# sailist/emotion-recognition-in-conversation

Measured on AMD Instinct MI355X. Metric: utterances/sec training step, COGMEN IEMOCAP-6 atv, higher is better.
Workload: dtype bf16

## Files before the change

emotion-recognition-in-conversation_amd/csrc/cogmen_fused.hip:

```cpp
#include "erc_common.h"
#include "split_dev.h"
#include "store_dev.h"

namespace {

typedef float f32x4 __attribute__((ext_vector_type(4)));
typedef short bf16x8 __attribute__((ext_vector_type(8)));

constexpr int CG_F = 100;
constexpr int CG_R = 8;
constexpr int CG_HL = 5;
constexpr int CG_TR = 16;
constexpr int CG_MID = CG_TR + 2 * CG_HL;
constexpr int CG_OUT = CG_TR + 4 * CG_HL;
constexpr int CG_FAR = CG_TR + 6 * CG_HL;
constexpr int CG_KM = (CG_R + 1) * CG_F;
constexpr int CG_KMP = 928;
constexpr int CG_SM = 936;
constexpr int CG_SH1 = 136;
constexpr int CG_SQ = 404;
constexpr int CG_CH = 12;
constexpr int CG_NT = 7;

constexpr int CG_NW = 16;
// ... 533 lines not shown
#pragma unroll
                for (int kb = 0; kb < 4; ++kb) {
                    sp_u32x4 fa0[NT], fa1[NT], fb[NT];
#pragma unroll
                    for (int t = 0; t < NT; ++t) {
                        const unsigned short* const pl = sH1 + t * (FW_SH1_BYTES / 2) + 32 * kb + 8 * g;
                        fa0[t] = *reinterpret_cast<const sp_u32x4*>(pl + r * CG_SH1), fa1[t] = *reinterpret_cast<const sp_u32x4*>(pl + (16 + r) * CG_SH1);
                        fb[t] = fqx[kb][t];
                        if (j == 0 && NT == 2) fqx[kb][t] = *reinterpret_cast<const sp_u32x4*>(bq1 + t * p.q_plane + 512 * kb);
                    }
                    acc[0] = sp_mfma<NT>(fa0, fb, acc[0]);
                    acc[1] = sp_mfma<NT>(fa1, fb, acc[1]);
                }
                if (j == 0 && NT > 2) {
                    __builtin_amdgcn_sched_barrier(0);
#pragma unroll
                    for (int kb = 0; kb < 4; ++kb)
#pragma unroll
                        for (int t = 0; t < NT; ++t) fqx[kb][t] = *reinterpret_cast<const sp_u32x4*>(bq1 + t * p.q_plane + 512 * kb);
                }
            } else {
#pragma unroll
            for (int kb = 0; kb < 4; ++kb)
#pragma unroll
                for (int h = 0; h < 2; ++h) acc[h] = __builtin_amdgcn_mfma_f32_16x16x32_bf16(fa[h][kb], fq[j][kb], acc[h], 0, 0, 0);
            }
            if (qt < 25) {
#pragma unroll
                for (int h = 0; h < 2; ++h)
#pragma unroll
                    for (int i = 0; i < 4; ++i) {
                        const int e = 16 * h + 4 * g + i;
                        if (e < CG_MID) sQ[e * CG_SQ + 16 * qt + r] = acc[h][i] + qbias[j];
                    }
            }
        }
    }
    __syncthreads();
    CG_STAMP(4);

#pragma unroll
    for (int j = 0; j < 2; ++j) {
        const int i = tid + CG_NTH * j;
        const int li = i / 100, q = i % 100;
        const int node = r0 + li;
        if (i < CG_TR * 100 && node < N)
            st_out16(p.QKVS + (int64_t)node * 400 + 4 * q, *reinterpret_cast<const f32x4*>(sQ + (CG_HL + li) * CG_SQ + 4 * q), p.wt);
    }

    {
        const bool act = lane < CG_F / 2;
        const int c2 = 2 * min(lane, CG_F / 2 - 1);
        const float am = act ? 1.f : 0.f;
        const int li = w, node = r0 + li, e = CG_HL + li;
        const bool valid = node < N;
        const int e0 = __builtin_amdgcn_readfirstlane(max(sIp[e] - E_lo, 0));
        const int nwin = __builtin_amdgcn_readfirstlane(valid ? min(max(sIp[e + 1] - sIp[e], 0), CG_CH) : 0);
        float2 qv = *reinterpret_cast<const float2*>(sQ + e * CG_SQ + c2);
        qv.x *= am, qv.y *= am;
        const float2 sk = *reinterpret_cast<const float2*>(sQ + e * CG_SQ + 3 * CG_F + c2);
        int ljs[CG_CH];
#pragma unroll
        for (int u = 0; u < CG_CH; ++u) ljs[u] = closed ? sSrc[e] + min(u, max(nwin - 1, 0)) : sSrc[min(e0 + min(u, max(nwin - 1, 0)), FW_ECAP - 1)];
        float2 kv[CG_CH], vv[CG_CH];
#pragma unroll
        for (int u = 0; u < CG_CH; ++u) {
            const float* row = sQ + min(max(ljs[u] - mb, 0), CG_MID - 1) * CG_SQ;
            kv[u] = *reinterpret_cast<const float2*>(row + CG_F + c2), vv[u] = *reinterpret_cast<const float2*>(row + 2 * CG_F + c2);
        }
        float sc[CG_CH], part[16];
#pragma unroll
        for (int u = 0; u < 16; ++u) part[u] = u < CG_CH ? qv.x * kv[u < CG_CH ? u : 0].x + qv.y * kv[u < CG_CH ? u : 0].y : 0.f;
        wave_sums_ch(part, sc, lane);
        float mx = -INFINITY, den = 0.f, o0 = 0.f, o1 = 0.f;
#pragma unroll
        for (int u = 0; u < CG_CH; ++u) {
            sc[u] *= p.scale;
            if (u < nwin) mx = fmaxf(mx, sc[u]);
        }
#pragma unroll
        for (int u = 0; u < CG_CH; ++u) {
            const float pw = u < nwin ? expf(sc[u] - mx) : 0.f;
            sc[u] = pw;
            den += pw;
            o0 += pw * vv[u].x, o1 += pw * vv[u].y;
        }
        const float inv = 1.0f / (den + 1e-16f);
        const float2 y = make_float2(valid ? o0 * inv + sk.x : 0.f, valid ? o1 * inv + sk.y : 0.f);
        if (act) *reinterpret_cast<float2*>(sH2 + li * CG_F + c2) = y;
        if (valid) {
            if (act && !p.h2_rows) *reinterpret_cast<float2*>(p.H2 + (int64_t)node * p.ldh2 + c2) = y;
            float mine = 0.f;
#pragma unroll
            for (int u = 0; u < CG_CH; ++u)
                if (lane == u) mine = sc[u];
            if (lane < nwin) p.alpha[sIp[e] + lane] = mine * inv;
        }
    }
    CG_STAMP(5);
    if (!p.bn_fused) return;

    __syncthreads();
    if (p.h2_rows && tid >= 512 && tid < 512 + CG_TR * (CG_F / 4)) {
        const int li = (tid - 512) / (CG_F / 4), q = (tid - 512) % (CG_F / 4);
        const int node = r0 + li;
        if (node < N) st_out16(p.H2 + (int64_t)node * p.ldh2 + 4 * q, *reinterpret_cast<const f32x4*>(sH2 + li * CG_F + 4 * q), p.wt);
    }
    if (tid < 2 * CG_F) {
        const int c = tid % CG_F, sq = tid / CG_F;
        double s = 0.0;
#pragma unroll
        for (int li = 0; li < CG_TR; ++li) {
            const double x = (double)sH2[li * CG_F + c];
            s += sq ? x * x : x;
        }
        if (p.bn_fused == 2) {
            reinterpret_cast<float*>(p.bn_part)[(int64_t)blockIdx.x * 2 * CG_F + tid] = (float)s;
        } else {
            st_sc1d(p.bn_part + (int64_t)blockIdx.x * 2 * CG_F + tid, s);
        }
    }
    if (p.bn_fused == 2) {
        CG_STAMP(6);
        return;
    }
    asm volatile("s_waitcnt vmcnt(0)" ::: "memory");
    __syncthreads();
    CG_STAMP(6);
    if (tid == 0) {
        const int prev = __hip_atomic_fetch_add(p.bn_counter, 1, __ATOMIC_RELAXED, __HIP_MEMORY_SCOPE_AGENT);
        const int last = prev == (int)gridDim.x - 1;
        if (last) __hip_atomic_store(p.bn_counter, 0, __ATOMIC_RELAXED, __HIP_MEMORY_SCOPE_AGENT);
        *s_last = last;
    }
    __syncthreads();
    if (!*s_last) return;
    {
        const int slot = tid & 255, part = tid >> 8;
        const int G = (int)gridDim.x, Gq = (G + 3) >> 2;
        const int g_begin = min(part * Gq, G), g_end = min(G, g_begin + Gq);
        double s = 0.0;
        if (slot < 2 * CG_F) {
            for (int g0 = g_begin; g0 < g_end; g0 += 32) {
                double t[32];
#pragma unroll
                for (int j = 0; j < 32; ++j) t[j] = ld_sc1d(p.bn_part + (int64_t)min(g0 + j, G - 1) * 2 * CG_F + slot);
#pragma unroll
                for (int j = 0; j < 32; ++j) s += t[j] * (g0 + j < g_end ? 1.0 : 0.0);
            }
        }
        sRed[part * 256 + slot] = s;
        __syncthreads();
        if (tid < CG_F) {
            const int c = tid;
            const double sx = ((sRed[c] + sRed[256 + c]) + sRed[512 + c]) + sRed[768 + c];
            const double sxx = ((sRed[CG_F + c] + sRed[256 + CG_F + c]) + sRed[512 + CG_F + c]) + sRed[768 + CG_F + c];
            const double m = sx / (double)N;
            double var = sxx / (double)N - m * m;
            if (var < 0.0) var = 0.0;
            p.saved[c] = (float)m;
            p.saved[CG_F + c] = (float)(1.0 / sqrt(var + (double)p.eps));
            const double unbiased = N > 1 ? var * (double)N / (double)(N - 1) : var;
            p.running_mean[c] = (1.f - p.momentum) * p.running_mean[c] + p.momentum * (float)m;
            p.running_var[c] = (1.f - p.momentum) * p.running_var[c] + p.momentum * (float)unbiased;
        }
        if (p.stamps && tid == 0) p.stamps[7] = __builtin_amdgcn_s_memrealtime();
    }
}

template <int CTRL>
__device__ __forceinline__ float cg_dpp(float v) {
    return __builtin_bit_cast(float, __builtin_amdgcn_update_dpp(0, __builtin_bit_cast(int, v), CTRL, 0xF, 0xF, true));
}
__device__ __forceinline__ float cg_row16_sum(float v) {
    v += cg_dpp<0xB1>(v), v += cg_dpp<0x4E>(v), v += cg_dpp<0x141>(v), v += cg_dpp<0x140>(v);
    return v;
}

constexpr int BW_ROWS = 48;
constexpr int BW_SK_OFF = 0;
constexpr int BW_SK_BYTES = BW_ROWS * CG_F * 4;
constexpr int BW_SV_OFF = BW_SK_OFF + BW_SK_BYTES;
constexpr int BW_SQ_OFF = BW_SV_OFF + BW_SK_BYTES;
constexpr int BW_SQ_BYTES = BW_ROWS * CG_F * 4;
constexpr int BW_BAND = 68;
constexpr int BW_SG_OFF = BW_SQ_OFF + BW_SQ_BYTES;
constexpr int BW_SE_OFF = BW_SG_OFF + BW_SQ_BYTES;
constexpr int BW_ECAP = 400;
constexpr int BW_OCAP = 288;
constexpr int BW_SE_BYTES = (3 * BW_ECAP + 4 * BW_OCAP + 40 + 28) * 4;
constexpr int BW_SDQ_OFF = BW_SE_OFF + ((BW_SE_BYTES + 15) / 16) * 16;
constexpr int CG_SDQ = 424;
constexpr int BW_SDQ_BYTES = 32 * CG_SDQ * 2;
constexpr int BW_SDH1_OFF = BW_SDQ_OFF + BW_SDQ_BYTES;
constexpr int BW_SDH1_BYTES = 32 * CG_F * 4;
constexpr int BW_SDP_OFF = BW_SDH1_OFF + BW_SDH1_BYTES;
constexpr int BW_SDP_BYTES = CG_TR * 968 * 2;
constexpr int BW_LDS = BW_SDP_OFF + BW_SDP_BYTES;
constexpr int CG_KB = 936;
constexpr int CG_KBP = 960;
constexpr int CG_SDP = 968;
static_assert(CG_TR * CG_SDP * 2 <= BW_SDP_BYTES && BW_SDP_OFF % 16 == 0 && BW_LDS <= 160 * 1024, "backward LDS map");
static_assert(2 * BW_ROWS * BW_BAND * 4 <= BW_SDP_BYTES, "the two band matrices live in the dP tile's area until the dP stage");
static_assert(3 * 4 * 2 * 64 * 4 * 4 <= BW_SDQ_BYTES, "K-split partials of the band product live in the dQKVS tile's area");

constexpr int BX_DQ_ROWS = CG_MID + 1;
constexpr int BX_DQPLANE = BX_DQ_ROWS * CG_SDQ * 2;
constexpr int BX_CP = 528;
constexpr int BX_DPPLANE = CG_TR * BX_CP * 2;
constexpr int BX_ZERO = 2 * 520;
template <int NT> constexpr int BX_PF = 3;
constexpr int BX_SE_BYTES16 = ((BW_SE_BYTES + 15) / 16) * 16;
template <int NT>
struct BxMap {
    static constexpr int SK_OFF = 0, SQ_OFF = BW_SK_BYTES, SG_OFF = 2 * BW_SK_BYTES;
    static constexpr int SE_OFF = 3 * BW_SK_BYTES;
    static constexpr int BAND_OFF = SE_OFF + BX_SE_BYTES16;
    static constexpr int BAND_BYTES = 2 * BW_ROWS * BW_BAND * 4;
    static constexpr int SV_OFF = BAND_OFF + BAND_BYTES;
    static constexpr int E_OFF = SV_OFF + BW_SK_BYTES;
    static constexpr int E_BYTES = NT * BX_DQPLANE - BW_SK_BYTES > 24576 ? NT * BX_DQPLANE - BW_SK_BYTES : 24576;
    static constexpr int LUT_OFF = E_OFF + E_BYTES;
    static constexpr int LDS = LUT_OFF + 1024;
    static_assert(NT * BX_DPPLANE <= 3 * BW_SK_BYTES && BW_SDH1_BYTES + 7 * 64 * 4 * 4 <= BAND_BYTES && LDS <= 160 * 1024 && SV_OFF % 16 == 0 &&
                      E_OFF % 16 == 0, "split backward LDS map");
};

struct CgBwdP {
    const float* dY;
    const float* H2;
    const float* gamma;
    const float* saved;
    const float* bn_bwd;
    const float* QKVS;
    const float* alpha;
    const int32_t* in_ptr;
    const int32_t* in_src;
    const int32_t* out_ptr;
    const int32_t* out_dst;
    const int32_t* out_typ;
    const int32_t* out_eid;
    const float* inv_cnt;
    const int32_t* node_spk;
    const float* head_part;
    float* bn_bwd_out;
    float* dgamma;
    float* dbeta;
    float* stats;
    int head_parts, hp_floats;
    const unsigned short* WqT;
    const unsigned short* Wb;
    float* dQKVS;
    float* dH1;
    float* dH0;
    float scale;
    int N, ldh2, lddh0, lddh1, grads_bf16, two_spk;
    const int32_t* n_dev;
    uint64_t* stamps;
    int stamp_block;
    int64_t qT_plane, wb_plane;
    int wt, dq_rows, dh1_rows;
    const int32_t* node_rec;
    int wp, wf;
};

template <int NT, bool CL>
__global__ __launch_bounds__(CG_NTH) void cogmen_bwd_tile_kernel(const CgBwdP p) {
    constexpr bool X = NT > 1;
    using XM = BxMap<X ? NT : 2>;
    extern __shared__ __attribute__((aligned(16))) unsigned char lds[];
    float* const sK = reinterpret_cast<float*>(lds + (X ? XM::SK_OFF : BW_SK_OFF));
    float* const sV = reinterpret_cast<float*>(lds + (X ? XM::SV_OFF : BW_SV_OFF));
    float* const sQq = reinterpret_cast<float*>(lds + (X ? XM::SQ_OFF : BW_SQ_OFF));
    float* const sG = reinterpret_cast<float*>(lds + (X ? XM::SG_OFF : BW_SG_OFF));
    float* const sAl = reinterpret_cast<float*>(lds + (X ? XM::SE_OFF : BW_SE_OFF));
    int* const sSrc = reinterpret_cast<int*>(sAl + 2 * BW_ECAP);
    int* const sOd = sSrc + BW_ECAP;
    int* const sOt = sOd + 2 * BW_OCAP;
    float* const sOw = reinterpret_cast<float*>(sOt + BW_OCAP);
    int* const sIp = reinterpret_cast<int*>(sOw + BW_OCAP);
    int* const sOp = sIp + 40;
    int* const sSpkOwn = reinterpret_cast<int*>(sAl + BW_ECAP);
    unsigned short* const sDQ = reinterpret_cast<unsigned short*>(lds + (X ? XM::SV_OFF : BW_SDQ_OFF));
    float* const sDH1 = reinterpret_cast<float*>(lds + (X ? XM::BAND_OFF : BW_SDH1_OFF));
    unsigned short* const sDP = reinterpret_cast<unsigned short*>(lds + (X ? XM::SK_OFF : BW_SDP_OFF));
    float* const sPart3 = sK;
    float* const sPart5 = X ? reinterpret_cast<float*>(lds + XM::BAND_OFF + BW_SDH1_BYTES) : sG;
    uint32_t* const sLut = reinterpret_cast<uint32_t*>(lds + XM::LUT_OFF);
    const int tid = threadIdx.x, lane = tid & 63, r = lane & 15, g = lane >> 4;
    const int w = __builtin_amdgcn_readfirstlane(tid >> 6);
    const int N = p.n_dev ? min(max(*p.n_dev, 1), p.N) : p.N;
    const int r0 = (int)blockIdx.x * CG_TR;
    const int mb = r0 - CG_HL, ob = r0 - 2 * CG_HL, fb = r0 - 3 * CG_HL;
    const int c1 = min(lane + 64, CG_F - 1);
    const bool h1 = lane + 64 < CG_F;
    const int ct = w & 7, kh = w >> 3;
    const bool mma_wave = ct < CG_NT;
    CG_STAMP(0);

    const int o_lo_node = min(max(ob, 0), N), o_hi_node = min(max(ob + CG_OUT, 0), N);
    const int m_lo_node = min(max(mb, 0), N), m_hi_node = min(max(mb + CG_MID, 0), N);
    constexpr bool closed = CL;
    int E_lo, E_hi, O_lo = 0, O_hi = 0;
    if constexpr (closed) {
        E_lo = p.node_rec[4 * (int64_t)o_lo_node + 2], E_hi = min(p.node_rec[4 * (int64_t)o_hi_node + 2], E_lo + BW_ECAP);
        if (tid < CG_OUT + 1) {
            const int nc = min(max(ob + tid, 0), N);
            const int4 rec = *reinterpret_cast<const int4*>(p.node_rec + 4 * (int64_t)nc);
            sIp[tid] = rec.z, sSrc[tid] = nc - min(rec.x, p.wf), sOd[tid] = rec.x, sOd[64 + tid] = rec.y;
        }
        if (tid >= 64 && tid < 64 + CG_OUT) {
            const int node = ob + tid - 64;
            const int sp = p.node_spk[min(max(node, 0), N - 1)];
            sOt[tid - 64] = (node >= 0 && node < N) ? sp : -1;
        }
    } else {
        E_lo = p.in_ptr[o_lo_node], E_hi = min(p.in_ptr[o_hi_node], E_lo + BW_ECAP);
        O_lo = p.out_ptr[m_lo_node], O_hi = min(p.out_ptr[m_hi_node], O_lo + BW_OCAP);
        if (tid < CG_OUT + 1) sIp[tid] = p.in_ptr[min(max(ob + tid, 0), N)];
        if (tid >= 64 && tid < 64 + CG_MID + 1) sOp[tid - 64] = p.out_ptr[min(max(mb + tid - 64, 0), N)];
    }
    if (tid >= 128 && tid < 128 + CG_TR) sSpkOwn[tid - 128] = p.node_spk[min(r0 + tid - 128, N - 1)];
    double* const sHp = reinterpret_cast<double*>(lds + (X ? XM::E_OFF : BW_SDQ_OFF));
    float* const sBnB = reinterpret_cast<float*>(lds + (X ? XM::E_OFF : BW_SDQ_OFF) + 4 * 256 * 8);
    if constexpr (X) {
        if (tid >= 768 && tid < 1024) {
            const int k4 = 4 * (tid - 768), q = k4 / 104, within = k4 - q * 104;
            uint32_t e = 3u << 16;
            if (q < CG_R) e = (uint32_t)(2 * ((q & 3) * 104 + within)) | ((1u + (uint32_t)(q >> 2)) << 16);
            else if (q == CG_R) e = (uint32_t)(2 * (4 * 104 + within));
            sLut[tid - 768] = e;
        }
    }
    if (p.head_part) {
        const int slot = tid & 255, part = tid >> 8;
        const int G = p.head_parts, Gq = (G + 3) >> 2;
        const int g_begin = min(part * Gq, G), g_end = min(G, g_begin + Gq);
        double acc = 0.0;
        if (slot < p.hp_floats) {
            for (int g0 = g_begin; g0 < g_end; g0 += 16) {
                float t[16];
#pragma unroll
                for (int j = 0; j < 16; ++j) t[j] = p.head_part[(int64_t)min(g0 + j, G - 1) * p.hp_floats + slot];
#pragma unroll
                for (int j = 0; j < 16; ++j) acc += (double)t[j] * (g0 + j < g_end ? 1.0 : 0.0);
            }
        }
        sHp[part * 256 + slot] = acc;
    }
    {
#pragma unroll
        for (int j = 0; j < 3; ++j) {
            const int i = tid + CG_NTH * j;
            const int f = min(i / 50, BW_ROWS - 1), q = i % 50;
            const int node = fb + f;
            const bool ok = f < CG_FAR && node >= 0 && node < N;
            const f32x4 v = *reinterpret_cast<const f32x4*>(p.QKVS + (int64_t)min(max(node, 0), N - 1) * 400 + CG_F + 4 * q);
            const float m = ok ? 1.f : 0.f;
            float* dst = (q < 25 ? sK + f * CG_F + 4 * q : sV + f * CG_F + 4 * (q - 25));
            if (i < BW_ROWS * 50) *reinterpret_cast<f32x4*>(dst) = (f32x4){v.x * m, v.y * m, v.z * m, v.w * m};
        }
        if (tid < BW_ECAP) {
            const int ei = min(E_lo + tid, max(E_hi - 1, E_lo));
            const bool ok = E_lo + tid < E_hi;
            const float a = p.alpha[ei];
            sAl[tid] = ok ? a : 0.f;
            if (!closed) {
                const int sj = p.in_src[ei];
                sSrc[tid] = ok ? sj : 0;
            }
        }
        if (!closed && tid >= 512 && tid < 512 + BW_OCAP) {
            const int i = tid - 512;
            const int oi = min(O_lo + i, max(O_hi - 1, O_lo));
            const bool ok = O_lo + i < O_hi;
            const int dst = p.out_dst[oi], typ = p.out_typ[oi];
            const float wgt = p.inv_cnt[(int64_t)dst * CG_R + min(typ, CG_R - 1)];
            sOd[i] = ok ? dst : 0;
            sOt[i] = ok ? typ : CG_R;
            sOw[i] = (ok && typ < CG_R) ? wgt : 0.f;
        }
    }
    f32x4 r_q[2], r_dy[2], r_x[2];
#pragma unroll
    for (int j = 0; j < 2; ++j) {
        const int i = tid + CG_NTH * j;
        const int e = min(i / 25, BW_ROWS - 1), q = i % 25;
        const int64_t nc = min(max(ob + e, 0), N - 1);
        r_q[j] = *reinterpret_cast<const f32x4*>(p.QKVS + nc * 400 + 4 * q);
        r_dy[j] = *reinterpret_cast<const f32x4*>(p.dY + nc * CG_F + 4 * q);
        r_x[j] = *reinterpret_cast<const f32x4*>(p.H2 + nc * p.ldh2 + 4 * q);
    }
    if (p.head_part) {
        __syncthreads();
        if (tid < 228) {
            const double sv = ((sHp[tid] + sHp[256 + tid]) + sHp[512 + tid]) + sHp[768 + tid];
            if (tid < 224) sBnB[tid] = (float)(sv / (double)N);
            if (blockIdx.x == 0) {
                const int c = tid < 112 ? tid : tid - 112;
                if (tid < 112 && c < CG_F) p.dbeta[c] = (float)sv, p.bn_bwd_out[c] = (float)(sv / (double)N);
                if (tid >= 112 && tid < 224 && c < CG_F) p.dgamma[c] = (float)sv, p.bn_bwd_out[CG_F + c] = (float)(sv / (double)N);
                const double wsum = ((sHp[226] + sHp[256 + 226]) + sHp[512 + 226]) + sHp[768 + 226];
                const double wmean = wsum / (double)p.head_parts;
                if (tid == 224) p.stats[0] = (float)(sv / wmean), p.stats[2] = (float)wmean;
                if (tid == 225) p.stats[1] = (float)sv;
            }
        }
        __syncthreads();
    }
#pragma unroll
    for (int j = 0; j < 2; ++j) {
        const int i = tid + CG_NTH * j;
        const int e = min(i / 25, BW_ROWS - 1), q = i % 25;
        const int node = ob + e;
        const bool ok = e < CG_OUT && node >= 0 && node < N;
        const f32x4 mu = *reinterpret_cast<const f32x4*>(p.saved + 4 * q), rs = *reinterpret_cast<const f32x4*>(p.saved + CG_F + 4 * q);
        const f32x4 ga = *reinterpret_cast<const f32x4*>(p.gamma + 4 * q);
        const f32x4 ma = p.head_part ? *reinterpret_cast<const f32x4*>(sBnB + 4 * q) : *reinterpret_cast<const f32x4*>(p.bn_bwd + 4 * q);
        const f32x4 mbv = p.head_part ? *reinterpret_cast<const f32x4*>(sBnB + 112 + 4 * q) : *reinterpret_cast<const f32x4*>(p.bn_bwd + CG_F + 4 * q);
        const float m = ok ? 1.f : 0.f;
        f32x4 gq, qq;
#pragma unroll
        for (int t = 0; t < 4; ++t) {
            gq[t] = ga[t] * rs[t] * (r_dy[j][t] - ma[t] - (r_x[j][t] - mu[t]) * rs[t] * mbv[t]) * m;
            qq[t] = r_q[j][t] * m;
        }
        if (i < BW_ROWS * 25) {
            *reinterpret_cast<f32x4*>(sG + e * CG_F + 4 * q) = gq;
            *reinterpret_cast<f32x4*>(sQq + e * CG_F + 4 * q) = qq;
        }
    }
    __syncthreads();
    CG_STAMP(1);

    float* const sDS = reinterpret_cast<float*>(lds + (X ? XM::BAND_OFF : BW_SDP_OFF));
    float* const sAL = sDS + BW_ROWS * BW_BAND;
    float* const sPartA = reinterpret_cast<float*>(lds + (X ? XM::E_OFF : BW_SDQ_OFF));
    {
        const int bi = w >> 2, bj = w & 3;
        f32x4 dA0 = {0.f, 0.f, 0.f, 0.f}, dA1 = {0.f, 0.f, 0.f, 0.f};
        if (bi < 3) {
            const float* const ga = sG + (16 * bi + r) * CG_F + g;
            const float* const v0 = sV + min(16 * bi + r, BW_ROWS - 1) * CG_F + g;
            const float* const v1 = sV + min(16 * (bi + 1) + r, BW_ROWS - 1) * CG_F + g;
            const int ks0 = 7 * bj, ks1 = min(25, ks0 + 7);
#pragma unroll
            for (int u = 0; u < 7; ++u) {
                const int ks = min(ks0 + u, 24);
                const float m = ks0 + u < ks1 ? 1.f : 0.f;
                const float af = ga[4 * ks] * m;
                dA0 = __builtin_amdgcn_mfma_f32_16x16x4f32(af, v0[4 * ks], dA0, 0, 0, 0);
                dA1 = __builtin_amdgcn_mfma_f32_16x16x4f32(af, v1[4 * ks], dA1, 0, 0, 0);
            }
            float* dst = sPartA + (((bi * 4 + bj) * 2) * 64 + lane) * 4;
            *reinterpret_cast<f32x4*>(dst) = dA0, *reinterpret_cast<f32x4*>(dst + 256) = dA1;
        } else {
            for (int i = lane + 64 * (w - 12); i < 2 * BW_ROWS * BW_BAND / 4; i += 256) reinterpret_cast<f32x4*>(sDS)[i] = (f32x4){0.f, 0.f, 0.f, 0.f};
        }
        __syncthreads();
        if (bi < 3) {
            const int q = bj;
            float a0 = 0.f, a1 = 0.f;
#pragma unroll
            for (int jj = 0; jj < 4; ++jj) {
                const float* src = sPartA + (((bi * 4 + jj) * 2) * 64 + lane) * 4 + q;
                a0 += src[0], a1 += src[256];
            }
            const int t = 16 * bi + 4 * g + q;
            const int node_t = ob + t;
            const bool tv = t < CG_OUT && node_t >= 0 && node_t < N;
            const int tc = min(t, CG_OUT - 1);
            const int e0 = min(max(sIp[tc] - E_lo, 0), BW_ECAP - 1);
            const int cnt = tv ? min(max(sIp[tc + 1] - sIp[tc], 0), CG_CH) : 0;
            const int lo = sSrc[closed ? tc : e0];
            const int o0 = (fb + 16 * bi + r) - lo, o1 = o0 + 16;
            const bool k0 = o0 >= 0 && o0 < cnt, k1 = o1 >= 0 && o1 < cnt;
            const float al0 = k0 ? sAl[min(e0 + max(o0, 0), BW_ECAP - 1)] : 0.f;
            const float al1 = k1 ? sAl[min(e0 + max(o1, 0), BW_ECAP - 1)] : 0.f;
            const float x0 = k0 ? al0 * a0 : 0.f, x1 = k1 ? al1 * a1 : 0.f;
            const float tsum = cg_row16_sum(x0 + x1);
            const float d0 = k0 ? al0 * (a0 - tsum) * p.scale : 0.f, d1 = k1 ? al1 * (a1 - tsum) * p.scale : 0.f;
            float* drow = sDS + t * BW_BAND + 16 * bi + r;
            float* arow = sAL + t * BW_BAND + 16 * bi + r;
            drow[0] = d0, drow[16] = d1;
            arow[0] = al0, arow[16] = al1;
        }
        __syncthreads();
    }
    CG_STAMP(2);

    const unsigned short* const brow3 = p.WqT + ((int64_t)(min(ct, CG_NT - 1) * 13 + 7 * kh) * 64 + lane) * 8;
    bf16x8 fb3[X ? 1 : 7];
    sp_u32x4 fb3r[X ? BX_PF<NT> : 1][X ? NT : 1], bxr[X ? BX_PF<NT> : 1][X ? NT : 1];
    if constexpr (!X) {
#pragma unroll
        for (int u = 0; u < 7; ++u) fb3[u] = *reinterpret_cast<const bf16x8*>(brow3 + 512 * min(u, kh ? 5 : 6));
    } else {
#pragma unroll
        for (int u = 0; u < BX_PF<NT>; ++u)
#pragma unroll
            for (int t = 0; t < NT; ++t) fb3r[u][t] = *reinterpret_cast<const sp_u32x4*>(brow3 + t * p.qT_plane + 512 * min(u, kh ? 5 : 6));
    }

    const unsigned short* const brow5 = p.Wb + ((int64_t)(min(ct, CG_NT - 1) * 30 + 15 * kh) * 64 + lane) * 8;
    bf16x8 bx[X ? 1 : 15];
    {
        uint32_t* const sDQw = reinterpret_cast<uint32_t*>(sDQ);
        constexpr int DQPW = BX_DQPLANE / 4;
        if constexpr (!X) {
            if (tid < CG_MID * 12) sDQw[(tid / 12) * (CG_SDQ / 2) + 200 + (tid % 12)] = 0u;
            for (int i = tid; i < 6 * (CG_SDQ / 2); i += CG_NTH) sDQw[CG_MID * (CG_SDQ / 2) + i] = 0u;
        } else {
#pragma unroll
            for (int t = 0; t < NT; ++t) {
                if (tid < CG_MID * 12) sDQw[t * DQPW + (tid / 12) * (CG_SDQ / 2) + 200 + (tid % 12)] = 0u;
                if (tid >= 512 && tid < 512 + CG_SDQ / 2) sDQw[t * DQPW + CG_MID * (CG_SDQ / 2) + tid - 512] = 0u;
            }
        }
#pragma unroll
        for (int j = 0; j < 2; ++j) {
            const int i = tid + CG_NTH * j;
            const int em = i / 50, cp = i % 50;
            if (i < CG_MID * 50) {
                const float2 gv = *reinterpret_cast<const float2*>(sG + (em + CG_HL) * CG_F + 2 * cp);
                if constexpr (!X) {
                    sDQw[em * (CG_SDQ / 2) + 150 + cp] = (uint32_t)f2bf(gv.x) | ((uint32_t)f2bf(gv.y) << 16);
                } else {
                    unsigned tt[NT];
                    sp_split2<NT>(gv.x, gv.y, tt);
#pragma unroll
                    for (int t = 0; t < NT; ++t) sDQw[t * DQPW + em * (CG_SDQ / 2) + 150 + cp] = tt[t];
                }
                const int node = mb + em;
                if ((X || !p.dq_rows) && em >= CG_HL && em < CG_HL + CG_TR && node < N) {
                    if (p.grads_bf16) *reinterpret_cast<uint32_t*>(reinterpret_cast<unsigned short*>(p.dQKVS) + (int64_t)node * 400 + 3 * CG_F + 2 * cp) = (uint32_t)f2bf(gv.x) | ((uint32_t)f2bf(gv.y) << 16);
                    else *reinterpret_cast<float2*>(p.dQKVS + (int64_t)node * 400 + 3 * CG_F + 2 * cp) = gv;
                }
            }
        }
#pragma unroll
        for (int ui = 0; ui < 3; ++ui) {
            if constexpr (!X) {
#pragma unroll
                for (int t5 = 0; t5 < 5; ++t5) bx[5 * ui + t5] = *reinterpret_cast<const bf16x8*>(brow5 + 512 * (5 * ui + t5));
            }
            const int u = w + CG_NW * ui;
            if (u >= 42) continue;
            const int kind = u < 14 ? 0 : 1 + (u - 14) / 14, uu = u < 14 ? u : (u - 14) % 14;
            const int rt = uu / 7, cti = uu % 7;
            const int col = min(16 * cti + r, CG_F - 1);
            f32x4 acc = {0.f, 0.f, 0.f, 0.f};
            if (kind == 0) {
                const float* const a = sDS + (16 * rt + r) * BW_BAND + 16 * rt + g;
                const float* const bq = sK + (16 * rt + g) * CG_F + col;
#pragma unroll
                for (int ks = 0; ks < 8; ++ks)
                    acc = __builtin_amdgcn_mfma_f32_16x16x4f32(a[4 * ks], bq[4 * ks * CG_F], acc, 0, 0, 0);
            } else {
                const float* const a = (kind == 1 ? sDS : sAL) + (16 * rt + g) * BW_BAND + 16 * rt + r + 2 * CG_HL;
                const float* const bq = (kind == 1 ? sQq : sG) + (16 * rt + g) * CG_F + col;
#pragma unroll
                for (int ks = 0; ks < 8; ++ks) acc = __builtin_amdgcn_mfma_f32_16x16x4f32(a[4 * ks * BW_BAND], bq[4 * ks * CG_F], acc, 0, 0, 0);
            }
            const int coff = kind * CG_F;
#pragma unroll
            for (int q = 0; q < 4; ++q) {
                const int em = kind == 0 ? 16 * rt + 4 * g + q - CG_HL : 16 * rt + 4 * g + q;
                const int node = mb + em;
                const bool rowv = em >= 0 && em < CG_MID;
                if (rowv && 16 * cti + r < CG_F) {
                    const bool nv = node >= 0 && node < N;
                    if constexpr (!X) {
                        sDQ[em * CG_SDQ + coff + 16 * cti + r] = f2bf(nv ? acc[q] : 0.f);
                    } else {
                        float rem = nv ? acc[q] : 0.f;
#pragma unroll
                        for (int t = 0; t < NT; ++t) {
                            const __bf16 hb = (__bf16)rem;
                            rem -= (float)hb;
                            sDQ[t * (BX_DQPLANE / 2) + em * CG_SDQ + coff + 16 * cti + r] = __builtin_bit_cast(unsigned short, hb);
                        }
                    }
                    if ((X || !p.dq_rows) && nv && em >= CG_HL && em < CG_HL + CG_TR) {
                        if (p.grads_bf16) reinterpret_cast<unsigned short*>(p.dQKVS)[(int64_t)node * 400 + coff + 16 * cti + r] = f2bf(acc[q]);
                        else p.dQKVS[(int64_t)node * 400 + coff + 16 * cti + r] = acc[q];
                    }
                }
            }
        }
    }
    __syncthreads();
    CG_STAMP(3);

    if constexpr (!X) {
        if (p.dq_rows && tid < CG_TR * 50) {
            static_assert((CG_SDQ * 2) % 16 == 0 && CG_TR * 50 <= CG_NTH, "row pieces of the dQKVS tile");
            const int li = tid / 50, q = tid % 50;
            const int node = r0 + li;
            if (node < N)
                st_out16(reinterpret_cast<unsigned short*>(p.dQKVS) + (int64_t)node * 400 + 8 * q,
                         *reinterpret_cast<const f32x4*>(sDQ + (CG_HL + li) * CG_SDQ + 8 * q), p.wt);
        }
    }

    {
        f32x4 acc0 = {0.f, 0.f, 0.f, 0.f}, acc1 = {0.f, 0.f, 0.f, 0.f};
        if (mma_wave) {
            const unsigned short* const a0 = sDQ + r * CG_SDQ + 8 * g + 32 * 7 * kh;
            if constexpr (!X) {
#pragma unroll
            for (int u = 0; u < 7; ++u) {
                if (u < (kh ? 6 : 7)) {
                    const bf16x8 fa0 = *reinterpret_cast<const bf16x8*>(a0 + 32 * u);
                    const bf16x8 fa1 = *reinterpret_cast<const bf16x8*>(a0 + 16 * CG_SDQ + 32 * u);
                    acc0 = __builtin_amdgcn_mfma_f32_16x16x32_bf16(fa0, fb3[u], acc0, 0, 0, 0);
                    acc1 = __builtin_amdgcn_mfma_f32_16x16x32_bf16(fa1, fb3[u], acc1, 0, 0, 0);
                }
            }
            } else {
                const int nkb3 = kh ? 6 : 7;
                const unsigned short* const a1 = sDQ + min(16 + r, CG_MID) * CG_SDQ + 8 * g + 32 * 7 * kh;
#pragma unroll
                for (int u = 0; u < 7; ++u) {
                    if (u < nkb3) {
                        sp_u32x4 fa0[NT], fa1[NT], fb[NT];
#pragma unroll
                        for (int t = 0; t < NT; ++t) {
                            fa0[t] = *reinterpret_cast<const sp_u32x4*>(a0 + t * (BX_DQPLANE / 2) + 32 * u);
                            fa1[t] = *reinterpret_cast<const sp_u32x4*>(a1 + t * (BX_DQPLANE / 2) + 32 * u);
                            fb[t] = fb3r[u % BX_PF<NT>][t];
                            if (u + BX_PF<NT> < 7) fb3r[u % BX_PF<NT>][t] = *reinterpret_cast<const sp_u32x4*>(brow3 + t * p.qT_plane + 512 * min(u + BX_PF<NT>, nkb3 - 1));
                        }
                        acc0 = sp_mfma<NT>(fa0, fb, acc0);
                        acc1 = sp_mfma<NT>(fa1, fb, acc1);
                    }
                }
                __builtin_amdgcn_sched_barrier(0);
#pragma unroll
                for (int u = 0; u < BX_PF<NT>; ++u)
#pragma unroll
                    for (int t = 0; t < NT; ++t) bxr[u][t] = *reinterpret_cast<const sp_u32x4*>(brow5 + t * p.wb_plane + 512 * u);
            }
            if (kh) {
                float* dst = sPart3 + (ct * 64 + lane) * 8;
                *reinterpret_cast<f32x4*>(dst) = acc0, *reinterpret_cast<f32x4*>(dst + 4) = acc1;
            }
        }
        __syncthreads();
        if (mma_wave && !kh) {
            const float* src = sPart3 + (ct * 64 + lane) * 8;
            const f32x4 p0 = *reinterpret_cast<const f32x4*>(src), p1 = *reinterpret_cast<const f32x4*>(src + 4);
            const int col = 16 * ct + r;
            if (col < CG_F) {
#pragma unroll
                for (int h = 0; h < 2; ++h)
#pragma unroll
                    for (int i = 0; i < 4; ++i) {
                        const int e = 16 * h + 4 * g + i;
                        const float v = h ? acc1[i] + p1[i] : acc0[i] + p0[i];
                        sDH1[e * CG_F + col] = v;
                        const int node = mb + e;
                        if ((X || !p.dh1_rows) && e >= CG_HL && e < CG_HL + CG_TR && node < N) {
                            if (p.grads_bf16) reinterpret_cast<unsigned short*>(p.dH1)[(int64_t)node * p.lddh1 + col] = f2bf(v);
                            else p.dH1[(int64_t)node * p.lddh1 + col] = v;
                        }
                    }
            }
        }
    }
    __syncthreads();
    CG_STAMP(4);

    if constexpr (!X) {
        if (p.dh1_rows && tid < CG_TR * 13) {
            const int li = tid / 13, q = tid % 13;
            const int node = r0 + li;
            const float* const src = sDH1 + (CG_HL + li) * CG_F + 8 * q;
            const f32x4 lo = *reinterpret_cast<const f32x4*>(src);
            f32x4 hi = {0.f, 0.f, 0.f, 0.f};
            if (q < 12) hi = *reinterpret_cast<const f32x4*>(src + 4);
            const uint32_t d0 = (uint32_t)f2bf(lo[0]) | ((uint32_t)f2bf(lo[1]) << 16), d1 = (uint32_t)f2bf(lo[2]) | ((uint32_t)f2bf(lo[3]) << 16);
            const uint32_t d2 = (uint32_t)f2bf(hi[0]) | ((uint32_t)f2bf(hi[1]) << 16), d3 = (uint32_t)f2bf(hi[2]) | ((uint32_t)f2bf(hi[3]) << 16);
            if (node < N)
                st_out16(reinterpret_cast<unsigned short*>(p.dH1) + (int64_t)node * p.lddh1 + 8 * q,
                         (f32x4){__builtin_bit_cast(float, d0), __builtin_bit_cast(float, d1), __builtin_bit_cast(float, d2), __builtin_bit_cast(float, d3)}, p.wt);
        }
    }

    {
        const bool act = lane < CG_F / 2;
        const int c2 = 2 * min(lane, CG_F / 2 - 1);
        uint32_t* const sDPw = reinterpret_cast<uint32_t*>(sDP);
        const int li = w, em = CG_HL + li, node = r0 + li;
        const bool valid = node < N;
        int nwin, my_off, my_typ;
        float my_w;
        if (closed) {
            const int to = 2 * CG_HL + li;
            const int pp = __builtin_amdgcn_readfirstlane(sOd[to]), L = __builtin_amdgcn_readfirstlane(sOd[64 + to]);
            const int klo = max(0, pp - p.wp);
            nwin = valid ? min(max(min(L - 1, pp + p.wf) - klo + 1, 0), CG_CH) : 0;
            const int my_spk = lane < CG_OUT ? sOt[lane] : -1;
            const unsigned long long mask0 = __ballot(my_spk == 0), mask1 = __ballot(my_spk == 1);
            const int b = __builtin_amdgcn_readfirstlane(min(max(sSpkOwn[li], 0), 1));
            const int kp = klo + min(lane, max(nwin - 1, 0));
            const int tk = min(max(to + kp - pp, CG_HL), CG_OUT - CG_HL - 1);
            const int dir = pp < kp ? 0 : 1;
            const int x0 = dir ? tk : tk - min(kp, p.wf), x1 = dir ? tk + min(p.wp, max(L - 1 - kp, 0)) + 1 : tk;
            const unsigned long long rm = x1 > x0 ? ((~0ull >> (64 - (x1 - x0))) << x0) : 0ull;
            const int c = __popcll((b ? mask1 : mask0) & rm);
            my_off = (tk - CG_HL) * CG_F;
            my_typ = lane < nwin ? 4 * b + 2 * min(max(sOt[tk], 0), 1) + dir : CG_R;
            my_w = c > 0 ? 1.0f / (float)c : 0.f;
        } else {
            const int o0 = __builtin_amdgcn_readfirstlane(sOp[em] - O_lo), o1 = __builtin_amdgcn_readfirstlane(sOp[em + 1] - O_lo);
            nwin = valid ? min(max(o1 - o0, 0), CG_CH) : 0;
            const int xb = max(o0, 0);
            const int xm = min(xb + min(lane, max(nwin - 1, 0)), BW_OCAP - 1);
            my_off = min(max(sOd[xm] - mb, 0), CG_MID - 1) * CG_F, my_typ = lane < nwin ? sOt[xm] : CG_R;
            my_w = sOw[xm];
        }
        float s0[CG_R], s1[CG_R];
#pragma unroll
        for (int q = 0; q < CG_R; ++q) s0[q] = s1[q] = 0.f;
        float t0[4] = {0.f, 0.f, 0.f, 0.f}, t1[4] = {0.f, 0.f, 0.f, 0.f};
        int b4 = 0;
        if (X || closed || p.two_spk) {
            b4 = 4 * __builtin_amdgcn_readfirstlane(min(max(sSpkOwn[li], 0), 1));
            float2 v[CG_CH];
            float wv[CG_CH];
            int gid[CG_CH];
#pragma unroll
            for (int u = 0; u < CG_CH; ++u) {
                const int uu = min(u, max(nwin - 1, 0));
                const int f = __builtin_amdgcn_readlane(my_off, uu);
                gid[u] = u < nwin ? __builtin_amdgcn_readlane(my_typ, uu) - b4 : -1;
                wv[u] = __builtin_bit_cast(float, __builtin_amdgcn_readlane(__builtin_bit_cast(int, my_w), uu));
                v[u] = *reinterpret_cast<const float2*>(sDH1 + f + c2);
            }
#pragma unroll
            for (int u = 0; u < CG_CH; ++u) {
                const float a0 = v[u].x * wv[u], a1 = v[u].y * wv[u];
                switch (gid[u]) {
                    case 0: t0[0] += a0, t1[0] += a1; break;
                    case 1: t0[1] += a0, t1[1] += a1; break;
                    case 2: t0[2] += a0, t1[2] += a1; break;
                    case 3: t0[3] += a0, t1[3] += a1; break;
                    default: break;
                }
            }
#pragma unroll
            for (int q = 0; q < CG_R; ++q) {
                const bool mine = (q & 4) == b4;
                s0[q] = mine ? t0[q & 3] : 0.f, s1[q] = mine ? t1[q & 3] : 0.f;
            }
        } else {
#pragma unroll 1
        for (int u = 0; u < nwin; u += 2) {
            const int u1 = min(u + 1, nwin - 1);
            const int f0 = __builtin_amdgcn_readlane(my_off, u), ty0 = __builtin_amdgcn_readlane(my_typ, u);
// ... 282 lines not shown
```

Baseline: 23.32 million.

## Hoist stage-0 global loads into registers ahead of LDS stores in backward kernel

Restructures the backward kernel's prologue so that all global loads (node records, speaker ids, K/V rows, Q/dY/H2 rows, the first block of head partials, alpha/src edges, BN saved/gamma constants) are issued early into registers. The LDS writes happen afterward, so memory latency overlaps instead of serialising behind each store. BN constants are staged once in LDS rather than re-read from global per thread, and the alpha/src LDS write is deferred past the first sync. The cost is higher register pressure from holding the 32 prefetched head partials and the other staged values, plus an extra unconditional barrier.

After: 23.51 million (median of 6 runs). No clear change (+0.8%).

```diff
diff --git a/emotion-recognition-in-conversation_amd/csrc/cogmen_fused.hip b/emotion-recognition-in-conversation_amd/csrc/cogmen_fused.hip
--- a/emotion-recognition-in-conversation_amd/csrc/cogmen_fused.hip
+++ b/emotion-recognition-in-conversation_amd/csrc/cogmen_fused.hip
@@ -859,27 +859,65 @@
     const int m_lo_node = min(max(mb, 0), N), m_hi_node = min(max(mb + CG_MID, 0), N);
     constexpr bool closed = CL;
     int E_lo, E_hi, O_lo = 0, O_hi = 0;
+    int4 n_rec = {0, 0, 0, 0};
+    int n_spk = 0, own_spk = 0;
     if constexpr (closed) {
         E_lo = p.node_rec[4 * (int64_t)o_lo_node + 2], E_hi = min(p.node_rec[4 * (int64_t)o_hi_node + 2], E_lo + BW_ECAP);
-        if (tid < CG_OUT + 1) {
-            const int nc = min(max(ob + tid, 0), N);
-            const int4 rec = *reinterpret_cast<const int4*>(p.node_rec + 4 * (int64_t)nc);
-            sIp[tid] = rec.z, sSrc[tid] = nc - min(rec.x, p.wf), sOd[tid] = rec.x, sOd[64 + tid] = rec.y;
-        }
-        if (tid >= 64 && tid < 64 + CG_OUT) {
-            const int node = ob + tid - 64;
-            const int sp = p.node_spk[min(max(node, 0), N - 1)];
-            sOt[tid - 64] = (node >= 0 && node < N) ? sp : -1;
-        }
+        if (tid < CG_OUT + 1) n_rec = *reinterpret_cast<const int4*>(p.node_rec + 4 * (int64_t)min(max(ob + tid, 0), N));
+        if (tid >= 64 && tid < 64 + CG_OUT) n_spk = p.node_spk[min(max(ob + tid - 64, 0), N - 1)];
     } else {
         E_lo = p.in_ptr[o_lo_node], E_hi = min(p.in_ptr[o_hi_node], E_lo + BW_ECAP);
         O_lo = p.out_ptr[m_lo_node], O_hi = min(p.out_ptr[m_hi_node], O_lo + BW_OCAP);
-        if (tid < CG_OUT + 1) sIp[tid] = p.in_ptr[min(max(ob + tid, 0), N)];
-        if (tid >= 64 && tid < 64 + CG_MID + 1) sOp[tid - 64] = p.out_ptr[min(max(mb + tid - 64, 0), N)];
-    }
-    if (tid >= 128 && tid < 128 + CG_TR) sSpkOwn[tid - 128] = p.node_spk[min(r0 + tid - 128, N - 1)];
+        if (tid < CG_OUT + 1) n_rec.x = p.in_ptr[min(max(ob + tid, 0), N)];
+        if (tid >= 64 && tid < 64 + CG_MID + 1) n_rec.y = p.out_ptr[min(max(mb + tid - 64, 0), N)];
+    }
+    if (tid >= 128 && tid < 128 + CG_TR) own_spk = p.node_spk[min(r0 + tid - 128, N - 1)];
+    constexpr int HB = 32;
+    const int h_slot = tid & 255, h_part = w >> 2;
+    const int h_G = p.head_parts, h_Gq = (h_G + 3) >> 2;
+    const int h_begin = min(h_part * h_Gq, h_G), h_end = min(h_G, h_begin + h_Gq);
+    const bool h_on = p.head_part && h_begin < h_end && h_slot < p.hp_floats;
+    const unsigned h_col = h_slot;
+    float h_t[HB];
+    if (h_on) {
+#pragma unroll
+        for (int j = 0; j < HB; ++j) h_t[j] = (p.head_part + (int64_t)min(h_begin + j, h_G - 1) * p.hp_floats)[h_col];
+    }
+    f32x4 r_kv[3];
+#pragma unroll
+    for (int j = 0; j < 3; ++j) {
+        const int i = tid + CG_NTH * j;
+        const int f = min(i / 50, BW_ROWS - 1), q = i % 50;
+        r_kv[j] = *reinterpret_cast<const f32x4*>(p.QKVS + (int64_t)min(max(fb + f, 0), N - 1) * 400 + CG_F + 4 * q);
+    }
+    f32x4 r_q[2], r_dy[2], r_x[2];
+#pragma unroll
+    for (int j = 0; j < 2; ++j) {
+        const int i = tid + CG_NTH * j;
+        const int e = min(i / 25, BW_ROWS - 1), q = i % 25;
+        const int64_t nc = min(max(ob + e, 0), N - 1);
+        r_q[j] = *reinterpret_cast<const f32x4*>(p.QKVS + nc * 400 + 4 * q);
+        r_dy[j] = *reinterpret_cast<const f32x4*>(p.dY + nc * CG_F + 4 * q);
+        r_x[j] = *reinterpret_cast<const f32x4*>(p.H2 + nc * p.ldh2 + 4 * q);
+    }
+    const int cq = min(max(tid - 512, 0), 74);
+    const f32x4 r_c = *reinterpret_cast<const f32x4*>(cq < 50 ? p.saved + 4 * cq : p.gamma + 4 * (cq - 50));
+
+    if constexpr (closed) {
+        if (tid < CG_OUT + 1) sIp[tid] = n_rec.z, sSrc[tid] = min(max(ob + tid, 0), N) - min(n_rec.x, p.wf), sOd[tid] = n_rec.x, sOd[64 + tid] = n_rec.y;
+        if (tid >= 64 && tid < 64 + CG_OUT) {
+            const int node = ob + tid - 64;
+            sOt[tid - 64] = (node >= 0 && node < N) ? n_spk : -1;
+        }
+    } else {
+        if (tid < CG_OUT + 1) sIp[tid] = n_rec.x;
+        if (tid >= 64 && tid < 64 + CG_MID + 1) sOp[tid - 64] = n_rec.y;
+    }
+    if (tid >= 128 && tid < 128 + CG_TR) sSpkOwn[tid - 128] = own_spk;
     double* const sHp = reinterpret_cast<double*>(lds + (X ? XM::E_OFF : BW_SDQ_OFF));
     float* const sBnB = reinterpret_cast<float*>(lds + (X ? XM::E_OFF : BW_SDQ_OFF) + 4 * 256 * 8);
+    float* const sBc = sBnB + 224;
+    static_assert(4 * 256 * 8 + (224 + 300) * 4 <= (X ? XM::E_BYTES : BW_SDQ_BYTES), "stage-0 scratch lives in the dQKVS tile's area");
     if constexpr (X) {
         if (tid >= 768 && tid < 1024) {
             const int k4 = 4 * (tid - 768), q = k4 / 104, within = k4 - q * 104;
@@ -889,22 +927,34 @@
             sLut[tid - 768] = e;
         }
     }
+    if (h_on) {
+#pragma unroll
+        for (int j = 0; j < HB; ++j) asm volatile("" : "+v"(h_t[j]));
+    }
+    float r_al = 0.f;
+    int r_src = 0;
+    const bool al_ok = E_lo + tid < E_hi;
+    if (tid < BW_ECAP) {
+        const int ei = min(E_lo + tid, max(E_hi - 1, E_lo));
+        r_al = p.alpha[ei];
+        if (!closed) r_src = p.in_src[ei];
+    }
     if (p.head_part) {
-        const int slot = tid & 255, part = tid >> 8;
-        const int G = p.head_parts, Gq = (G + 3) >> 2;
-        const int g_begin = min(part * Gq, G), g_end = min(G, g_begin + Gq);
         double acc = 0.0;
-        if (slot < p.hp_floats) {
-            for (int g0 = g_begin; g0 < g_end; g0 += 16) {
+        if (h_on) {
+#pragma unroll
+            for (int j = 0; j < HB; ++j) acc += (double)h_t[j] * (h_begin + j < h_end ? 1.0 : 0.0);
+            for (int g0 = h_begin + HB; g0 < h_end; g0 += 16) {
                 float t[16];
 #pragma unroll
-                for (int j = 0; j < 16; ++j) t[j] = p.head_part[(int64_t)min(g0 + j, G - 1) * p.hp_floats + slot];
-#pragma unroll
-                for (int j = 0; j < 16; ++j) acc += (double)t[j] * (g0 + j < g_end ? 1.0 : 0.0);
-            }
-        }
-        sHp[part * 256 + slot] = acc;
-    }
+                for (int j = 0; j < 16; ++j) t[j] = (p.head_part + (int64_t)min(g0 + j, h_G - 1) * p.hp_floats)[h_col];
+#pragma unroll
+                for (int j = 0; j < 16; ++j) acc += (double)t[j] * (g0 + j < h_end ? 1.0 : 0.0);
+            }
+        }
+        sHp[h_part * 256 + h_slot] = acc;
+    }
+    CG_STAMP(8);
     {
 #pragma unroll
         for (int j = 0; j < 3; ++j) {
@@ -912,21 +962,14 @@
             const int f = min(i / 50, BW_ROWS - 1), q = i % 50;
             const int node = fb + f;
             const bool ok = f < CG_FAR && node >= 0 && node < N;
-            const f32x4 v = *reinterpret_cast<const f32x4*>(p.QKVS + (int64_t)min(max(node, 0), N - 1) * 400 + CG_F + 4 * q);
+            const f32x4 v = r_kv[j];
             const float m = ok ? 1.f : 0.f;
             float* dst = (q < 25 ? sK + f * CG_F + 4 * q : sV + f * CG_F + 4 * (q - 25));
             if (i < BW_ROWS * 50) *reinterpret_cast<f32x4*>(dst) = (f32x4){v.x * m, v.y * m, v.z * m, v.w * m};
         }
-        if (tid < BW_ECAP) {
-            const int ei = min(E_lo + tid, max(E_hi - 1, E_lo));
-            const bool ok = E_lo + tid < E_hi;
-            const float a = p.alpha[ei];
-            sAl[tid] = ok ? a : 0.f;
-            if (!closed) {
-                const int sj = p.in_src[ei];
-                sSrc[tid] = ok ? sj : 0;
-            }
-        }
+    }
+    if (tid >= 512 && tid < 512 + 75) *reinterpret_cast<f32x4*>(sBc + 4 * (tid - 512)) = r_c;
+    {
         if (!closed && tid >= 512 && tid < 512 + BW_OCAP) {
             const int i = tid - 512;
             const int oi = min(O_lo + i, max(O_hi - 1, O_lo));
@@ -938,18 +981,8 @@
             sOw[i] = (ok && typ < CG_R) ? wgt : 0.f;
         }
     }
-    f32x4 r_q[2], r_dy[2], r_x[2];
-#pragma unroll
-    for (int j = 0; j < 2; ++j) {
-        const int i = tid + CG_NTH * j;
-        const int e = min(i / 25, BW_ROWS - 1), q = i % 25;
-        const int64_t nc = min(max(ob + e, 0), N - 1);
-        r_q[j] = *reinterpret_cast<const f32x4*>(p.QKVS + nc * 400 + 4 * q);
-        r_dy[j] = *reinterpret_cast<const f32x4*>(p.dY + nc * CG_F + 4 * q);
-        r_x[j] = *reinterpret_cast<const f32x4*>(p.H2 + nc * p.ldh2 + 4 * q);
-    }
+    __syncthreads();
     if (p.head_part) {
-        __syncthreads();
         if (tid < 228) {
             const double sv = ((sHp[tid] + sHp[256 + tid]) + sHp[512 + tid]) + sHp[768 + tid];
             if (tid < 224) sBnB[tid] = (float)(sv / (double)N);
@@ -965,14 +998,15 @@
         }
         __syncthreads();
     }
+    CG_STAMP(9);
 #pragma unroll
     for (int j = 0; j < 2; ++j) {
         const int i = tid + CG_NTH * j;
         const int e = min(i / 25, BW_ROWS - 1), q = i % 25;
         const int node = ob + e;
         const bool ok = e < CG_OUT && node >= 0 && node < N;
-        const f32x4 mu = *reinterpret_cast<const f32x4*>(p.saved + 4 * q), rs = *reinterpret_cast<const f32x4*>(p.saved + CG_F + 4 * q);
-        const f32x4 ga = *reinterpret_cast<const f32x4*>(p.gamma + 4 * q);
+        const f32x4 mu = *reinterpret_cast<const f32x4*>(sBc + 4 * q), rs = *reinterpret_cast<const f32x4*>(sBc + CG_F + 4 * q);
+        const f32x4 ga = *reinterpret_cast<const f32x4*>(sBc + 2 * CG_F + 4 * q);
         const f32x4 ma = p.head_part ? *reinterpret_cast<const f32x4*>(sBnB + 4 * q) : *reinterpret_cast<const f32x4*>(p.bn_bwd + 4 * q);
         const f32x4 mbv = p.head_part ? *reinterpret_cast<const f32x4*>(sBnB + 112 + 4 * q) : *reinterpret_cast<const f32x4*>(p.bn_bwd + CG_F + 4 * q);
         const float m = ok ? 1.f : 0.f;
@@ -987,6 +1021,7 @@
             *reinterpret_cast<f32x4*>(sQq + e * CG_F + 4 * q) = qq;
         }
     }
+    CG_STAMP(10);
     __syncthreads();
     CG_STAMP(1);
 
@@ -1013,6 +1048,10 @@
             *reinterpret_cast<f32x4*>(dst) = dA0, *reinterpret_cast<f32x4*>(dst + 256) = dA1;
         } else {
             for (int i = lane + 64 * (w - 12); i < 2 * BW_ROWS * BW_BAND / 4; i += 256) reinterpret_cast<f32x4*>(sDS)[i] = (f32x4){0.f, 0.f, 0.f, 0.f};
+        }
+        if (tid < BW_ECAP) {
+            sAl[tid] = al_ok ? r_al : 0.f;
+            if (!closed) sSrc[tid] = al_ok ? r_src : 0;
         }
         __syncthreads();
         if (bi < 3) {
```
